# inferflow/inferflow

Measured on AMD Instinct MI355X. Metric: decode tokens/sec, Llama-2-7B Q4 batch=1 greedy (whole job), higher is better.
Workload: dtype i8 (Q8 activations x Q4_B32T1A weights, i32 dot, f32 scale, f16 I/O); 1 GPU; llama2_7b decode, Q4_B32T1A weights + F16 lm_head, F16 KV cache, batch 1 greedy, 16-token prompt, context 21..1851; parallelism=single, weights_bytes=4309647360

## Files before the change

inferflow_amd/csrc/ifa_decode_chain.h:

```cpp
#pragma once
#include "ifa_decode_kernels.h"

namespace ifa {

struct DecChainExtra {
    uint32_t *gran_a;
    uint32_t *gran_h;
    uint32_t *flags_a, *flags_h;
    const int *state;
    const unsigned *epoch;
    unsigned epoch_add;
    unsigned *err;
    int timeout_us;
    long long *trace;
    int late_w2;
};

__device__ __forceinline__ uint32_t chain_tag(unsigned call, int pos) { return 0x8000u | ((call & 127u) << 8) | ((unsigned)pos & 255u); }

typedef uint32_t ch_u32x4 __attribute__((ext_vector_type(4)));

template <int MAXC>
__device__ __forceinline__ bool chain_gather(half8_t (&xv)[MAXC], const uint32_t *gran, int cols, int nthr, uint32_t tag,
                                             long long t_give_up, unsigned *err, unsigned code)
// ... 152 lines not shown
        typename FmtA::W wo[RO];
        const int rows_o = PW.total_rows;
#pragma unroll
        for (int i = 0; i < RO; i++) {
            const int v = i * W + gw;
            if (i > 0 && v >= rows_o) continue;
            wo[i].load(PW.W0[0] + (size_t)min(v, rows_o - 1) * row_bytes_a, nblk_a, lane);
        }
        const half_t res = PW.residual[min(min(lane, RO - 1) * W + gw, rows_o - 1)];
        zero_ctl();
        read_tag();
        if (trf) { trc[0] = t_kernel; trc[1] = wall_clock64(); }
        __syncthreads();
        float aw[RO];
#pragma unroll
        for (int i = 0; i < RO; i++) aw[i] = (i == 0 || i * W + gw < rows_o) ? wo[i].dot(XA) : 0.0f;
#pragma unroll
        for (int i = 0; i < RO; i++) aw[i] = wave_sum(aw[i]);
        float a0 = 0.0f;
#pragma unroll
        for (int i = 0; i < RO; i++) { if (lane == i) a0 = aw[i]; }
        const int v = lane * W + gw;
        if (lane < RO && v < rows_o) {
            const DecRow d = dec_locate(PW, v);
            const half_t y = dec_row_value<EPI_RESIDUAL>(PW, d, a0, 0.0f, res, (half_t)0);
            chain_publish(E.gran_a, d.row, tag, y);
            d.y[d.row] = y;
        }
        chain_wave_published(ctl + CH_C_PUB_A, NW, E.flags_a + blockIdx.x, tag, lane);
        if (trf) trc[2] = wall_clock64();
        if (trl) trc[0] = wall_clock64();
        if (wave >= NP) {
            load_rows13(0, 0, RW);
        } else {
            if (wave == 0) { chain_poll_flags(E.flags_a, G, tag, lane, t_give_up, E.err, 0x93u); chain_go(ctl + CH_C_GO_A); }
            else lds_counter_wait(ctl + CH_C_GO_A, 1);
            chain_gather<MAXC>(pre.xv, E.gran_a, pcols, PT, tag, t_give_up, E.err, 0x91u);
            if (trf) trc[3] = wall_clock64();
            pre.finish(P.norm_w, P.norm_b, P.multi_base, P.eps, pcols, L, nullptr, nullptr);
            load_rows13(0, 0, RW);
        }
        lds_counter_wait(L.part + 131, NP);
    } else {
        if (threadIdx.x < PT) pre.issue(px, pnw, pnb, pcols);
        zero_ctl();
        if (NORM == 1 && wave >= NP) load_rows13(0, 0, 1);
        read_tag();
// ... 75 lines not shown
        else res = Q.residual[row];
        if (Q.residual2) res2 = Q.residual2[row];
    }
    if (trl) trc[3] = wall_clock64();
    lds_counter_wait(L2.part + 131, NP);
    if (trl) trc[4] = wall_clock64();
    if (lw >= rows2) return;
    float a2[R2];
#pragma unroll
    for (int i = 0; i < R2; i++) a2[i] = 0.0f;
#pragma unroll
    for (int j = 0; j < NJB; j++) {
        typename Fmt1::X Xj;
        Xj.load(L2.codes, L2.scale, L2.xsum, lane, nblk_b, 64 * j);
#pragma unroll
        for (int i = 0; i < R2; i++) a2[i] = (i == 0 || i * WL + lw < rows2) ? w2[i][j].dot(Xj, a2[i]) : 0.0f;
    }
#pragma unroll
    for (int i = 0; i < R2; i++) a2[i] = wave_sum(a2[i]);
    float b0 = 0.0f;
#pragma unroll
    for (int i = 0; i < R2; i++) { if (lane == i) b0 = a2[i]; }
    const int v2 = lane * WL + lw;
    if (lane < R2 && v2 < rows2) dec_finish_row<EPI_RESIDUAL>(Q, dec_locate(Q, v2), b0, 0.0f, res, res2);
    if (trl) trc[5] = wall_clock64();
}

bool dec_chain_supported(int w_dtype, int w2_dtype, int wo_dtype, int dim, int ffn, bool wo, int wo_cols, int num_cus);
int dec_chain_launch(int w_dtype, bool glu, int norm, bool wo, const DecGemvParams &P, const DecGemvParams &Q, const DecGemvParams *PW,
                     const DecChainExtra &E, int num_cus, hipStream_t s);
template <int DT>
int dec_chain_launch_dt(bool glu, int norm, bool wo, const DecGemvParams &P, const DecGemvParams &Q, const DecGemvParams &PW,
                        const DecChainExtra &E, int num_cus, hipStream_t s);

}
```

inferflow_amd/csrc/ifa_decode_kernels.h:

```cpp
#pragma once
#include "ifa_device.h"
#include "ifa_math.h"
#include "ifa_tiled.h"
#include "ifa_decode_formats.h"
#include "ifa_decode_gemv_plan.h"

namespace ifa {

typedef _Float16 half2_t __attribute__((ext_vector_type(2)));
typedef _Float16 half8_t __attribute__((ext_vector_type(8)));

__device__ __forceinline__ void q8_round_div8(const float (&v)[8], float qs, int (&q)[8])
{
    const float rqs = 1.0f / qs;
    bool risky = false;
#pragma unroll
    for (int i = 0; i < 8; i++) {
        const float t = v[i] * rqs;
        const float k = __builtin_rintf(t);
        risky |= fabsf(fabsf(t - k) - 0.5f) < 0.00006103515625f;
        q[i] = (int)k;
    }
    if (__builtin_expect(risky, 0)) {
#pragma unroll
// ... 6 lines not shown
#pragma unroll
    for (int i = 0; i < 8; i++) q[i] = min(max(q[i], -128), 127);
}

__device__ __forceinline__ int q8_round_div1(float v, float qs)
{
    if (qs <= 0.000001f) return 0;
    const float t = v * (1.0f / qs);
    float k = __builtin_rintf(t);
    if (__builtin_expect(fabsf(fabsf(t - k) - 0.5f) < 0.00006103515625f, 0)) k = roundf(v / qs);
    return min(max((int)k, -128), 127);
}

__device__ __forceinline__ void q8x4_dequant_h(uint32_t w, half2_t sc2, half2_t &lo, half2_t &hi)
{
    const uint32_t x = w ^ 0x80808080u;
    const uint32_t a = __builtin_amdgcn_perm(0x64646464u, x, 0x04010400u);
    const uint32_t b = __builtin_amdgcn_perm(0x64646464u, x, 0x04030402u);
    const half2_t bias = {(half_t)-1152.0f, (half_t)-1152.0f};
    lo = (__builtin_bit_cast(half2_t, a) + bias) * sc2;
    hi = (__builtin_bit_cast(half2_t, b) + bias) * sc2;
}

#ifndef IFA_NT_WEIGHTS
#define IFA_NT_WEIGHTS 1
#endif

struct XLds {
    int8_t *codes;
    float *scale;
    float *xsum;
    float *part;
    half_t *xh;
};


__device__ __forceinline__ XLds xlds_carve(char *smem, int cols)
{
    XLds l;
    size_t nb = (size_t)cols / 32;
    size_t off = 0;
    l.codes = reinterpret_cast<int8_t *>(smem); off += ((size_t)cols + 15) / 16 * 16;
    l.scale = reinterpret_cast<float *>(smem + off); off += nb * 4;
    l.xsum = reinterpret_cast<float *>(smem + off); off += nb * 4;
    off = (off + 15) / 16 * 16;
    l.part = reinterpret_cast<float *>(smem + off); off += 132 * 4;
// ... 57 lines not shown
#pragma unroll
            for (int i = 0; i < 8; i++) {
                half_t t = av[k][i];
                if (add_bias) t = f2h(h2f(t) + h2f(abv[k][i]));
                xv[k][i] = f2h(h2f(xv[k][i]) + h2f(t));
            }
            if (sum_out && blockIdx.x == 0) *reinterpret_cast<half8_t *>(sum_out + (size_t)c * 8) = xv[k];
        }
    }

    __device__ __forceinline__ void issue(const half_t *__restrict__ x, const half_t *__restrict__ nw,
                                          const half_t *__restrict__ nb, int cols)
    {
        const int chunks = cols >> 3;
#pragma unroll
        for (int k = 0; k < MAXC; k++) {
            const int c = threadIdx.x + k * nthr();
            if (c < chunks) {
                xv[k] = *reinterpret_cast<const half8_t *>(x + (size_t)c * 8);
                if constexpr (NORM == 1) {
                    if (nw) wv[k] = *reinterpret_cast<const half8_t *>(nw + (size_t)c * 8);
                    if (nb) bv[k] = *reinterpret_cast<const half8_t *>(nb + (size_t)c * 8);
                }
            }
        }
    }

    __device__ __forceinline__ void issue_norm(const half_t *__restrict__ nw, const half_t *__restrict__ nb, int cols)
    {
        if constexpr (NORM == 1) {
            const int chunks = cols >> 3;
#pragma unroll
            for (int k = 0; k < MAXC; k++) {
                const int c = threadIdx.x + k * nthr();
                if (c < chunks) {
                    if (nw) wv[k] = *reinterpret_cast<const half8_t *>(nw + (size_t)c * 8);
                    if (nb) bv[k] = *reinterpret_cast<const half8_t *>(nb + (size_t)c * 8);
                }
            }
        }
    }

    __device__ __forceinline__ void finish(const half_t *__restrict__ nw, const half_t *__restrict__ nb,
                                           float multi_base, float eps, int cols, const XLds &L,
                                           half_t *__restrict__ xn_out, long long *trc = nullptr)
    {
// ... 206 lines not shown

struct DecRow {
    int si, row;
    const uint8_t *W0, *W1;
    const half_t *b0, *b1;
    half_t *y;
};

__device__ __forceinline__ DecRow dec_locate(const DecGemvParams &P, int v)
{
    const int r0 = P.rows[0], r1 = P.rows[1];
    DecRow d;
    const bool in1 = P.nsets > 1 && v >= r0;
    const bool in2 = P.nsets > 2 && v >= r0 + r1;
    d.si = in2 ? 2 : (in1 ? 1 : 0);
    d.row = in2 ? v - r0 - r1 : (in1 ? v - r0 : v);
    d.W0 = in2 ? P.W0[2] : (in1 ? P.W0[1] : P.W0[0]);
    d.W1 = P.W1;
    d.b0 = in2 ? P.b0[2] : (in1 ? P.b0[1] : P.b0[0]);
    d.b1 = P.b1;
    d.y = in2 ? P.y[2] : (in1 ? P.y[1] : P.y[0]);
    return d;
}

template <int EPI>
__device__ __forceinline__ half_t dec_row_value(const DecGemvParams &P, const DecRow d, float a0, float a1, half_t res = (half_t)0,
                                                half_t res2 = (half_t)0)
{
    const int row = d.row;
    half_t y = dec_bias(a0, d.b0, row);
    if constexpr (EPI == EPI_RESIDUAL || EPI == EPI_PLAIN) {
        if (P.pre_scale != 0.0f) y = f2h(h2f(y) * P.pre_scale);
    }
    if constexpr (EPI == EPI_RESIDUAL) {
        y = f2h(h2f(res) + h2f(y));
        if (P.residual2) y = f2h(h2f(y) + h2f(res2));
        if (P.post_scale != 0.0f) y = f2h(h2f(y) * P.post_scale);
    } else if constexpr (EPI == EPI_GLU || EPI == EPI_MOE_GLU) {
        half_t t2 = dec_bias(a1, d.b1, row);
        half_t act = f2h(act_fn(h2f(y), P.act_kind));
        y = f2h(h2f(act) * h2f(t2));
    } else if constexpr (EPI == EPI_ACT || EPI == EPI_MOE_ACT) {
        y = f2h(act_fn(h2f(y), P.act_kind));
    } else if constexpr (EPI == EPI_MOE_ACC || EPI == EPI_MOE_LAST) {
        const half_t wexp = P.moe_w[P.moe_slot];
        const half_t prev = P.moe_slot == 0 ? (half_t)0 : P.moe_acc[row];
        y = __builtin_fmaf16(y, wexp, prev);
        if constexpr (EPI == EPI_MOE_LAST) {
            if (P.pre_scale != 0.0f) y = f2h(h2f(y) * P.pre_scale);
            y = f2h(h2f(y) + h2f(P.residual[row]));
            if (P.residual2) y = f2h(h2f(y) + h2f(P.residual2[row]));
            if (P.post_scale != 0.0f) y = f2h(h2f(y) * P.post_scale);
        }
    }
    return y;
}

template <int EPI>
__device__ __forceinline__ void dec_finish_row(const DecGemvParams &P, const DecRow d, float a0, float a1, half_t res = (half_t)0,
                                               half_t res2 = (half_t)0)
{
    d.y[d.row] = dec_row_value<EPI>(P, d, a0, a1, res, res2);
}

template <int DT, int NJ, int RW, int EPI, int NORM, bool XADD = false, int TH = DEC_THREADS, int NP = 0>
__global__ void __launch_bounds__(TH) k_dec_gemv(const half_t *px, const half_t *pnw, const half_t *pnb, int pcols,
                                                          const uint8_t *pw0, const uint8_t *pw1, int pnblk_grid, int ptotal,
                                                          const DecGemvParams P)
{
    extern __shared__ __attribute__((aligned(16))) char smem[];
    static_assert(NP == 0 || (NORM != 2 && !XADD && NP * 64 < TH), "wave-specialised prologue: a norm / quantiser prologue, some loader waves");
    constexpr int PT = NP ? NP * 64 : TH;
    constexpr int MAXC = NORM == 2 ? 1 : (NJ * 8 * block_capacity(DT) + PT - 1) / PT;
    XPre<NORM == 2 ? 0 : NORM, MAXC, XADD, NP * 64> pre;
    if constexpr (NORM != 2) {
        if (NP == 0 || threadIdx.x < PT) pre.issue(px, pnw, pnb, pcols);
        if constexpr (XADD) pre.issue_add(P.x_add, P.x_add_bias, pcols);
    }
    const long long t_start = wall_clock64();
    const XLds L = xlds_carve(smem, pcols);
    const int lane = threadIdx.x & 63;
    const int wave = __builtin_amdgcn_readfirstlane(threadIdx.x >> 6);
    const int gw = blockIdx.x * (TH / 64) + wave;
    const int W = (int)((unsigned)pnblk_grid >> 16) * (TH / 64);
    using Fmt = DecFmt<DT, NJ>;
    constexpr int NM = epi_is_glu(EPI) ? 2 : 1;
    const bool single = !epi_is_moe(EPI) && pw0 != nullptr;
    const int nblk_k = pnblk_grid & 0xFFFF, total_rows = ptotal;
    const size_t row_bytes = tiled_row_bytes(DT, (size_t)nblk_k);
    const int npass = (total_rows + RW * W - 1) / (RW * W);


    const uint8_t *moeW0 = nullptr, *moeW1 = nullptr, *moeW0b = nullptr, *moeW1b = nullptr, *moeW0c = nullptr, *moeW1c = nullptr;
    if constexpr (epi_is_moe(EPI)) {
        const int e = __builtin_amdgcn_readfirstlane(P.moe_sel[P.moe_slot]);
        moeW0 = P.w_table[4 * e + P.moe_tab_off];
        if constexpr (NM == 2) moeW1 = P.w_table[4 * e + P.moe_tab_off + 1];
        moeW0b = moeW0; moeW1b = moeW1; moeW0c = moeW0; moeW1c = moeW1;
        if (P.nsets > 1) {
            const int e1 = __builtin_amdgcn_readfirstlane(P.moe_sel[P.moe_slot + 1]);
            moeW0b = P.w_table[4 * e1 + P.moe_tab_off];
            if constexpr (NM == 2) moeW1b = P.w_table[4 * e1 + P.moe_tab_off + 1];
        }
        if (P.nsets > 2) {
            const int e2 = __builtin_amdgcn_readfirstlane(P.moe_sel[P.moe_slot + 2]);
            moeW0c = P.w_table[4 * e2 + P.moe_tab_off];
            if constexpr (NM == 2) moeW1c = P.w_table[4 * e2 + P.moe_tab_off + 1];
        }
    }
    auto moe_pick = [](int si, const uint8_t *a, const uint8_t *b, const uint8_t *c) { return si == 2 ? c : (si == 1 ? b : a); };
    typename Fmt::W w[NM][RW];
    auto load_rows = [&](int pass, int i0, int i1) {
        const bool full = (pass * RW + RW - 1) * W + gw < total_rows;
        auto one = [&](int i) {
            const int v = min((pass * RW + i) * W + gw, total_rows - 1);
            if (single) {
                w[0][i].load(pw0 + (size_t)v * row_bytes, nblk_k, lane);
                if constexpr (NM == 2) w[1][i].load(pw1 + (size_t)v * row_bytes, nblk_k, lane);
                return;
            }
            const DecRow d = dec_locate(P, v);
            const uint8_t *W0 = epi_is_moe(EPI) ? moe_pick(d.si, moeW0, moeW0b, moeW0c) : d.W0;
            w[0][i].load(W0 + (size_t)d.row * row_bytes, nblk_k, lane);
            if constexpr (NM == 2) { const uint8_t *W1 = epi_is_moe(EPI) ? moe_pick(d.si, moeW1, moeW1b, moeW1c) : d.W1; w[1][i].load(W1 + (size_t)d.row * row_bytes, nblk_k, lane); }
        };
        if (full) {
#pragma unroll
            for (int i = 0; i < RW; i++) { if (i < i0 || i >= i1) continue; one(i); }
        } else {
#pragma unroll
            for (int i = 0; i < RW; i++) {
                if (i < i0 || i >= i1) continue;
                if (i > 0 && (pass * RW + i) * W + gw >= total_rows) continue;
                one(i);
            }
        }
    };
    auto load_pass = [&](int pass) { load_rows(pass, 0, RW); };
    half_t res = (half_t)0, res2 = (half_t)0;
    auto load_epi = [&](int pass) {
        if constexpr (EPI == EPI_RESIDUAL) {
            const int v = min((pass * RW + min(lane, RW - 1)) * W + gw, total_rows - 1);
            const int row = single ? v : dec_locate(P, v).row;
            res = P.residual[row];
            if (P.residual2) res2 = P.residual2[row];
        }
    };
    constexpr int D1 = (NM * NJ * Fmt::DW >= 15) ? 1 : 2;

    typename Fmt::X X;
    bool tr = false;
    auto trace_on = [&]() { tr = P.trace != nullptr && threadIdx.x == 64; if (tr) P.trace[blockIdx.x * 8 + 0] = t_start; };
    if constexpr (NORM == 2) {
        const XqImage Q = xq_image_carve(const_cast<half_t *>(px), pcols);
        X.load(Q.codes, Q.scale, Q.xsum, lane, nblk_k);
        load_rows(0, 0, RW);
        load_epi(0);
        trace_on();
        if (tr) { P.trace[blockIdx.x * 8 + 1] = wall_clock64(); P.trace[blockIdx.x * 8 + 2] = wall_clock64(); }
        if (gw >= total_rows) return;
    } else {
        if constexpr (NP > 0) {
            if (threadIdx.x == TH - 1) { L.part[130] = 0.0f; L.part[131] = 0.0f; }
            constexpr int EARLY = NORM == 1 ? 1 : 0;
            if (EARLY && wave >= NP) load_rows(0, 0, 1);
            trace_on();
            __syncthreads();
            if (wave >= NP) {
                load_rows(0, EARLY, RW);
                load_epi(0);
                if (P.trace != nullptr && threadIdx.x == NP * 64 && NORM == 1) P.trace[blockIdx.x * 8 + 4] = wall_clock64();
            } else {
                if (tr) P.trace[blockIdx.x * 8 + 1] = wall_clock64();
                pre.finish(P.norm_w, P.norm_b, P.multi_base, P.eps, P.cols, L, P.xn_out,
                           (P.trace != nullptr && threadIdx.x == 0) ? P.trace + blockIdx.x * 8 : nullptr);
                load_rows(0, 0, RW);
                load_epi(0);
                if (tr) P.trace[blockIdx.x * 8 + 2] = wall_clock64();
            }
            lds_counter_wait(L.part + 131, NP);
        } else {
        __syncthreads();
        load_rows(0, 0, D1);
        trace_on();
        if (tr) P.trace[blockIdx.x * 8 + 1] = wall_clock64();
        if constexpr (XADD) pre.apply_add(P.x_add_bias, P.cols, P.xsum_out);
        pre.finish(P.norm_w, P.norm_b, P.multi_base, P.eps, P.cols, L, P.xn_out,
                   (P.trace != nullptr && threadIdx.x == 0) ? P.trace + blockIdx.x * 8 : nullptr);
        load_rows(0, D1, RW);
        load_epi(0);
        if (tr) P.trace[blockIdx.x * 8 + 2] = wall_clock64();
        }
        if (gw >= total_rows) return;
        X.load(L.codes, L.scale, L.xsum, lane, nblk_k);
    }
    if (tr) P.trace[blockIdx.x * 8 + 3] = wall_clock64();

    for (int pass = 0; pass < npass; pass++) {
        if (pass > 0) { load_pass(pass); load_epi(pass); }
        float a[NM][RW];
#pragma unroll
        for (int i = 0; i < RW; i++)
#pragma unroll
            for (int m = 0; m < NM; m++) a[m][i] = w[m][i].dot(X);
#pragma unroll
        for (int i = 0; i < RW; i++)
#pragma unroll
            for (int m = 0; m < NM; m++) a[m][i] = wave_sum(a[m][i]);
        float a0 = 0.0f, a1 = 0.0f;
#pragma unroll
        for (int i = 0; i < RW; i++) {
            if (lane == i) { a0 = a[0][i]; if constexpr (NM == 2) a1 = a[1][i]; }
        }
        const int v = (pass * RW + lane) * W + gw;
        if (lane < RW && v < total_rows) {
            dec_finish_row<EPI>(P, dec_locate(P, v), a0, a1, res, res2);
        }
    }
    if (tr) P.trace[blockIdx.x * 8 + 7] = wall_clock64();
}

template <int DT, int NJ, int RW, int EPI>
__global__ void __launch_bounds__(DEC_THREADS) k_dec_gemv_long(const DecGemvParams P)
{
    extern __shared__ __attribute__((aligned(16))) char smem[];
    const XLds L = xlds_carve(smem, P.cols);
    const int lane = threadIdx.x & 63;
    const int wave = __builtin_amdgcn_readfirstlane(threadIdx.x >> 6);
    const int gw = blockIdx.x * DEC_WAVES + wave;
    const int W = gridDim.x * DEC_WAVES;
    using Fmt = DecFmt<DT, NJ>;
    const size_t row_bytes = tiled_row_bytes(DT, (size_t)P.nblk);
    const int npass = (P.total_rows + RW * W - 1) / (RW * W);
    const int nchunk = (P.nblk + 64 * NJ - 1) / (64 * NJ);
    const int Q = npass * nchunk;
    const uint8_t *moeW0 = nullptr;
    if constexpr (epi_is_moe(EPI)) moeW0 = P.w_table[4 * __builtin_amdgcn_readfirstlane(P.moe_sel[P.moe_slot]) + P.moe_tab_off];
    typename Fmt::W wa[RW], wb[RW];
    auto load_q = [&](typename Fmt::W (&w)[RW], int q, int i0, int i1) {
        const int pass = q / nchunk, chunk = q - pass * nchunk;
#pragma unroll
        for (int i = 0; i < RW; i++) {
            if (i < i0 || i >= i1) continue;
            const int v = min((pass * RW + i) * W + gw, P.total_rows - 1);
            const DecRow d = dec_locate(P, v);
            const uint8_t *W0 = epi_is_moe(EPI) ? moeW0 : d.W0;
            w[i].load(W0 + (size_t)d.row * row_bytes, P.nblk, lane, chunk * 64 * NJ);
        }
    };
    {
        XPre<0, 8> pre;
        pre.issue(P.x, nullptr, nullptr, P.cols);
        __syncthreads();
        load_q(wa, 0, 0, 1);
        pre.finish(nullptr, nullptr, 0.0f, P.eps, P.cols, L, nullptr, nullptr);
        load_q(wa, 0, 1, RW);
    }
    if (gw >= P.total_rows) return;
    float a[RW];
#pragma unroll
    for (int i = 0; i < RW; i++) a[i] = 0.0f;
    auto compute = [&](typename Fmt::W (&w)[RW], int q) {
        const int pass = q / nchunk, chunk = q - pass * nchunk;
        typename Fmt::X X;
        X.load(L.codes, L.scale, L.xsum, lane, P.nblk, chunk * 64 * NJ);
#pragma unroll
        for (int i = 0; i < RW; i++) a[i] = w[i].dot(X, a[i]);
        if (chunk + 1 < nchunk) return;
#pragma unroll
        for (int i = 0; i < RW; i++) a[i] = wave_sum(a[i]);
        float a0 = 0.0f;
#pragma unroll
        for (int i = 0; i < RW; i++) { if (lane == i) a0 = a[i]; a[i] = 0.0f; }
        const int v = (pass * RW + lane) * W + gw;
        if (lane < RW && v < P.total_rows) {
            const DecRow d = dec_locate(P, v);
            half_t res = (half_t)0, res2 = (half_t)0;
            if constexpr (EPI == EPI_RESIDUAL) { res = P.residual[d.row]; if (P.residual2) res2 = P.residual2[d.row]; }
            dec_finish_row<EPI>(P, d, a0, 0.0f, res, res2);
        }
    };
    for (int q = 0; q < Q; q += 2) {
        if (q + 1 < Q) load_q(wb, q + 1, 0, RW);
        compute(wa, q);
        if (q + 1 < Q) {
            if (q + 2 < Q) load_q(wa, q + 2, 0, RW);
            compute(wb, q + 1);
        }
    }
}

struct DecLmHeadParams {
    const half_t *x;
    const half_t *norm_w, *norm_b;
    float multi_base, eps;
    int cols;
    const half_t *W;
    half_t *logits;
    int rows;
    half_t *xn_out;
};

// ... 177 lines not shown
```

inferflow_amd/csrc/ifa_dgemv_f16x.hip:

```cpp
#include "ifa_decode_gemv.h"
#include "ifa_codec.h"

namespace ifa {

constexpr int DH_ROWS = DEC_H_ROWS;

template <int DT>
struct HRow {
    const uint8_t *p;
    __device__ __forceinline__ float dot(const half_t *__restrict__ xs, int cols, int nblk, int lane) const
    {
        float acc = 0.0f;
        if constexpr (DT == F16) {
            const int chunks = cols >> 3;
            const u32x4 *w = reinterpret_cast<const u32x4 *>(p);
            const u32x4 *xv = reinterpret_cast<const u32x4 *>(xs);
            for (int c0 = lane; c0 < chunks; c0 += 256) {
                u32x4 wr[4];
#pragma unroll
                for (int j = 0; j < 4; j++) { const int c = c0 + 64 * j; wr[j] = w[min(c, chunks - 1)]; }
#pragma unroll
                for (int j = 0; j < 4; j++) { const int c = c0 + 64 * j; if (c < chunks) acc = dot8_f16(wr[j], xv[c], acc); }
            }
        } else {
// ... 57 lines not shown
            const int c = tid + k * DEC_THREADS;
            if (c >= chunks) continue;
            const half8_t v = *reinterpret_cast<const half8_t *>(xs + (size_t)c * 8);
            half8_t o;
#pragma unroll
            for (int i = 0; i < 8; i++) {
                float t = (float)v[i] * scale;
                if (P.norm_w) {
                    const float mlt = P.multi_base + h2f(P.norm_w[(size_t)c * 8 + i]);
                    t = t * mlt;
                    if (P.norm_b) t = t + h2f(P.norm_b[(size_t)c * 8 + i]);
                }
                o[i] = f2h(t);
            }
            *reinterpret_cast<half8_t *>(xs + (size_t)c * 8) = o;
            if (P.xn_out && blockIdx.x == 0) *reinterpret_cast<half8_t *>(P.xn_out + (size_t)c * 8) = o;
        }
        __syncthreads();
    }
    constexpr int NM = epi_is_glu(EPI) ? 2 : 1;
    const int gw = blockIdx.x * DEC_WAVES + wave;
    const int W = gridDim.x * DEC_WAVES;
    const size_t row_bytes = DT == F16 ? (size_t)P.cols * 2 : (size_t)P.nblk * block_bytes(DT);
    for (int v0 = gw; v0 < P.total_rows; v0 += DH_ROWS * W) {
        float a[NM][DH_ROWS];
#pragma unroll
        for (int i = 0; i < DH_ROWS; i++) {
            const int v = min(v0 + i * W, P.total_rows - 1);
            const DecRow d = dec_locate(P, v);
            HRow<DT> r0{d.W0 + (size_t)d.row * row_bytes};
            a[0][i] = r0.dot(xs, P.cols, P.nblk, lane);
            if constexpr (NM == 2) { HRow<DT> r1{d.W1 + (size_t)d.row * row_bytes}; a[1][i] = r1.dot(xs, P.cols, P.nblk, lane); }
        }
#pragma unroll
        for (int i = 0; i < DH_ROWS; i++)
#pragma unroll
            for (int mm = 0; mm < NM; mm++) a[mm][i] = wave_sum(a[mm][i]);
        float a0 = 0.0f, a1 = 0.0f;
#pragma unroll
        for (int i = 0; i < DH_ROWS; i++)
            if (lane == i) { a0 = a[0][i]; if constexpr (NM == 2) a1 = a[1][i]; }
        const int v = v0 + lane * W;
        if (lane < DH_ROWS && v < P.total_rows) {
            const DecRow d = dec_locate(P, v);
            half_t res = (half_t)0, res2 = (half_t)0;
            if constexpr (EPI == EPI_RESIDUAL) { res = P.residual[d.row]; if (P.residual2) res2 = P.residual2[d.row]; }
            dec_finish_row<EPI>(P, d, a0, a1, res, res2);
        }
    }
}

bool dec_gemv_h_supported(int w_dtype, size_t cols)
{
    return dec_gemv_h_cols_ok(w_dtype, cols);
}

DecGemvPlan dec_gemv_h_plan(const DecGemvFacts &f) { return plan_dec_gemv_h(f); }

template <int DT, int EPI, int NORM, bool XADD>
static int launch_h(const DecGemvParams &P, hipStream_t s)
{
    DecGemvFacts F;
    F.dtype = DT; F.epi = EPI; F.norm = NORM; F.x_add = XADD; F.cols = P.cols; F.total_rows = P.total_rows; F.num_cus = dec_num_cus();
    const DecGemvPlan R = plan_dec_gemv_h(F);
    if (R.error) return ifa_fail(IFA_ERR_ARG, "fused fp16-activation GEMV: dtype %d with %d columns is not supported", DT, P.cols);
    const size_t smem = (size_t)R.lds;
    const int wgs = R.grid;
    auto kern = k_dec_gemv_h<DT, EPI, NORM, XADD>;
    if (smem > 48 * 1024) IFA_HIP_CHECK(hipFuncSetAttribute((const void *)kern, hipFuncAttributeMaxDynamicSharedMemorySize, (int)smem));
    kern<<<dim3((unsigned)wgs), dim3(DEC_THREADS), smem, s>>>(P);
// ... 39 lines not shown
```

inferflow_amd/csrc/ifa_engine.hip:

```cpp
#include <mutex>
#include <unordered_map>
#include "ifa_engine_state.h"

namespace ifa {

namespace {
struct SpaceBook {
    std::mutex mu;
    std::unordered_map<void *, size_t> live;
    long long live_bytes = 0, fail_at = 0;
};
SpaceBook &book() { static SpaceBook *b = new SpaceBook(); return *b; }

template <class Alloc> int space_alloc(const char *call, void **p, size_t bytes, Alloc alloc)
{
    SpaceBook &b = book();
    *p = nullptr;
    {
        std::lock_guard<std::mutex> g(b.mu);
        if (b.fail_at > 0 && --b.fail_at == 0)
            return ifa_fail(IFA_ERR_HIP, "%s(%zu bytes) failed: out of memory (simulated: ifa_debug_alloc_fail_at)", call, bytes);
    }
    const hipError_t e = alloc(p, bytes);
    if (e != hipSuccess) {
// ... 89 lines not shown
        if (sl.exec) { (void)hipGraphExecDestroy(sl.exec); sl.exec = nullptr; }
        if (sl.graph) { (void)hipGraphDestroy(sl.graph); sl.graph = nullptr; }
    }
    for (auto &kv : m->batch_graphs) if (kv.second) (void)hipGraphExecDestroy(kv.second);
    m->batch_graphs.clear();
    for (auto &kv : m->draft_graphs) if (kv.second) (void)hipGraphExecDestroy(kv.second);
    m->draft_graphs.clear();
    sampled_drop_graphs(m);
}

int ensure_scratch(ifa_model *m, int T)
{
    if (T <= m->scratch_tokens) return IFA_OK;
    const ifa_model_config &c = m->cfg;
    const size_t D = c.dim, QD = (size_t)c.heads * c.head_dim, KVD = (size_t)c.kv_heads * c.head_dim, F = c.ffn;
    size_t maxcols = std::max(std::max(D, QD), F);
    Scratch n;
    int rc;
    if ((rc = n.x.alloc(T * D)) || (rc = n.x2.alloc(T * D)) || (rc = n.xn.alloc(T * D)) || (rc = n.hn.alloc(T * D)) || (rc = n.pn.alloc(T * D))
        || (rc = n.q.alloc(T * QD)) || (rc = n.k.alloc(T * KVD)) || (rc = n.v.alloc(T * KVD)) || (rc = n.att.alloc(T * QD))
        || (rc = n.a.alloc(T * D)) || (rc = n.f.alloc(T * D)) || (rc = n.t1.alloc(std::max<size_t>(T, 3) * F)) || (rc = n.t2.alloc(T * F))
        || (rc = n.logits.alloc((size_t)T * c.vocab)))
        return rc;
    if (!m->dqkv && (rc = n.dqkv.alloc(QD + 2 * KVD))) return rc;
    if (T <= 32 && !m->bqkv && ((rc = n.bqkv.alloc(32 * (QD + 2 * KVD))) || (rc = n.brope.alloc(32 * (size_t)c.head_dim)))) return rc;
    if (c.experts > 0) {
        const size_t cap = (size_t)T * (size_t)std::max(1, c.moe_top_k);
        if ((rc = n.moe_gate.alloc((size_t)T * c.experts)) || (rc = n.moe_out.alloc((size_t)T * D)) || (rc = n.moe_in.alloc((size_t)T * D))
            || (rc = n.moe_wdev.alloc(cap)) || (rc = n.moe_idx.alloc(cap)) || (rc = n.moe_pin.alloc(cap * (sizeof(int) + 2) + 16)))
            return rc;
        if (!m->moe_route) {
            if ((rc = n.moe_route.alloc(64 / sizeof(int)))) return rc;
            IFA_HIP_CHECK(hipMemsetAsync(n.moe_route, 0, 64, m->stream));
        }
        if ((rc = n.moe_sel.alloc(cap)) || (rc = n.moe_epos.alloc(cap)) || (rc = n.moe_counts.alloc(16))
            || (rc = n.moe_xq_in.alloc(cap * (D / 32 + 1) * 34)) || (rc = n.moe_xq_mid.alloc(cap * (F / 32 + 1) * 34))
            || (rc = n.moe_tiles.alloc((cap / 64 + (size_t)c.experts + 1) * sizeof(MoeTile)))
            || (rc = n.moe_singles.alloc(((size_t)c.experts + 1) * sizeof(MoeSingle))) || (rc = n.moe_smalls.alloc(((size_t)c.experts + 1) * sizeof(MoeTile)))
            || (rc = n.moe_selw.alloc(cap)) || (rc = n.moe_g1.alloc(cap * F)) || (rc = n.moe_g3.alloc(cap * F)) || (rc = n.moe_gin.alloc(cap * D))
            || (rc = n.moe_gout.alloc(cap * D)))
            return rc;
    }
    if ((rc = n.xq.alloc((maxcols / 32 + 1) * 34))) return rc;
    if (!m->attq && (rc = n.attq.alloc(xq_image_bytes(c.heads * c.head_dim)))) return rc;
    if ((rc = n.tokens_dev.alloc((size_t)T))) return rc;
    if (!n.dqkv) n.dqkv = std::move(m->dqkv);
    if (!n.bqkv) { n.bqkv = std::move(m->bqkv); n.brope = std::move(m->brope); }
// ... 447 lines not shown
}

int ifa_model_prompt_route(ifa_model *m, int *out, int n_out)
{
    IFA_REQUIRE(m && out && n_out >= PROMPT_ROUTE_N_OUT, "ifa_model_prompt_route: %d outputs expected", PROMPT_ROUTE_N_OUT);
    memcpy(out, &m->prompt_route, sizeof(m->prompt_route));
    return IFA_OK;
}

int ifa_model_get_buffer(ifa_model *m, const char *name, int layer, void **dptr, size_t *bytes)
{
    IFA_REQUIRE(m && name && dptr, "ifa_model_get_buffer: null pointer");
    const ifa_model_config &c = m->cfg;
    size_t b = 0; void *p = nullptr;
    if (!strcmp(name, "logits")) { p = m->logits; b = (size_t)c.vocab * 2; }
    else if (!strcmp(name, "logits_adj")) { p = m->la_adj; b = m->la_adj ? m->la_adj.cap() / m->g[T_LM_HEAD].rows * (size_t)c.vocab * 2 : 0; }
    else if (!strcmp(name, "logit_state")) { p = m->la_state; b = m->la_slots * m->g[T_LM_HEAD].rows * sizeof(unsigned); }
    else if (!strcmp(name, "tp_logits")) { p = m->tp_logits; b = m->tp_logits ? m->g[T_LM_HEAD].rows * 2 : 0; }
    else if (!strcmp(name, "trace")) { p = m->trace; b = m->trace ? sizeof(long long) * 2048 * 8 : 0; }
    else if (!strcmp(name, "hidden")) { p = m->xn; b = (size_t)c.dim * 2; }
    else if (!strcmp(name, "x")) { p = m->x; b = (size_t)c.dim * 2; }
    else if (!strcmp(name, "x2")) { p = m->x2; b = (size_t)c.dim * 2; }
    else if (!strcmp(name, "dqkv")) { p = m->dqkv; b = ((size_t)c.heads + 2 * (size_t)c.kv_heads) * c.head_dim * 2; }
    else if (!strcmp(name, "att")) { p = m->att; b = (size_t)c.heads * c.head_dim * 2; }
    else if (!strcmp(name, "attq")) { p = m->attq; b = m->attq ? xq_image_bytes(c.heads * c.head_dim) : 0; }
    else if (!strcmp(name, "a")) { p = m->a; b = (size_t)c.dim * 2; }
    else if (!strcmp(name, "t1")) { p = m->t1; b = (size_t)c.ffn * 2; }
    else if (!strcmp(name, "kcache") || !strcmp(name, "vcache")) {
        IFA_REQUIRE(layer >= 0 && layer < c.layers && m->finalized, "ifa_model_get_buffer: layer %d", layer);
        p = name[0] == 'k' ? m->layers[(size_t)layer].kcache : m->layers[(size_t)layer].vcache;
        b = m->kv_row_bytes * (size_t)c.max_ctx;
    } else return ifa_fail(IFA_ERR_ARG, "ifa_model_get_buffer: unknown buffer '%s'", name);
    *dptr = p;
    if (bytes) *bytes = b;
    return IFA_OK;
}

void *ifa_model_stream(ifa_model *m) { return m ? (void *)m->stream : nullptr; }

int ifa_model_set_stream(ifa_model *m, ifa_stream stream)
{
    IFA_REQUIRE(m, "ifa_model_set_stream: null model");
    IFA_HIP_CHECK(hipSetDevice(m->cfg.device));
    if (m->stream) IFA_HIP_CHECK(hipStreamSynchronize(m->stream));
    if (m->stream) (void)ifa_gemm_release_stream((ifa_stream)m->stream);
    if (m->stream && m->own_stream) IFA_HIP_CHECK(hipStreamDestroy(m->stream));
// ... 38 lines not shown
```

inferflow_amd/csrc/ifa_engine_state.h:

```cpp
#pragma once
#include <chrono>
#include <cstdlib>
#include <cstring>
#include <map>
#include <string>
#include <type_traits>
#include <vector>
#include "ifa_host.h"
#include "ifa_buf_hip.h"
#include "ifa_decode_kernels.h"
#include "ifa_decode_attn.h"
#include "ifa_decode_gemv.h"
#include "ifa_moe.h"
#include "ifa_gemm_rows_mfma.h"
#include "ifa_gemm_big.h"
#include "ifa_decode_lmhead_tail.h"
#include "ifa_decode_singles.h"
#include "ifa_decode_qkv_attn.h"
#include "ifa_decode_chain.h"
#include "ifa_prompt_route.h"

using namespace ifa;

namespace ifae {
// ... 6 lines not shown
       T_ATTN_POST_NORM = 29, T_ATTN_POST_NORM_B = 30, T_FFN_POST_NORM = 31, T_FFN_POST_NORM_B = 32,
       T_MAX = 36 };

struct Tensor {
    int dtype = -1;
    DevBuf<void> data;
    DevBuf<void> tiled;
    DevBuf<void> mo;
    DevBuf<void> q3hn;
    DevBuf<void> x32;
    size_t rows = 0, cols = 0;
    bool present() const { return data != nullptr; }
};

struct Layer {
    Tensor t[T_MAX];
    std::vector<Tensor> experts;
    DevBuf<void *> moe_table;
    DevBuf<void *> moe_table_aos;
    DevBuf<void *> moe_table_mo;
    DevBuf<void> kcache, vcache;
};

struct Scratch {
    DevBuf<half_t> x, x2, xn, hn, q, k, v;
    DevBuf<half_t> dqkv;
    DevBuf<half_t> bqkv;
    DevBuf<float> brope;
    DevBuf<half_t> att, a, f, t1, t2, logits;
    DevBuf<uint8_t> xq;
    DevBuf<int8_t> attq;
    DevBuf<half_t> moe_gate, moe_out;
    DevBuf<half_t> moe_in, moe_wdev;
    DevBuf<int> moe_route;
    DevBuf<int> moe_idx; PinBuf<void> moe_pin;
    DevBuf<int> moe_sel, moe_epos, moe_counts;
    DevBuf<half_t> moe_selw, moe_g1, moe_g3, moe_gin, moe_gout;
    DevBuf<uint8_t> moe_xq_in, moe_xq_mid;
    DevBuf<void> moe_tiles, moe_singles, moe_smalls;
    DevBuf<int> tokens_dev;
    DevBuf<half_t> pn;
};


}
using namespace ifae;
// ... 289 lines not shown
```

Baseline: 630.3 tokens/s.

## Read GEMV epilogue params from kernarg segment and branch-free row-set addressing

Reworks the decode GEMV epilogue and weight-row addressing. Parameters are read straight from the kernarg segment into scalar registers, and dec_locate is replaced with branch-free offset arithmetic. Bias and residual values are prefetched alongside the weight loads, and the unconditional clamped x issue (issue_all) removes per-chunk branches. It also adds a dqkv guard allocation so speculative reads stay in bounds, trace points, and a compile flag that disables the early-row prologue. The aim is to cut SGPR/VGPR pressure and the latency of the epilogue and prologue, at the cost of relying on a fixed kernarg layout and some extra clamped memory reads.

```diff
diff --git a/inferflow_amd/csrc/ifa_decode_chain.h b/inferflow_amd/csrc/ifa_decode_chain.h
--- a/inferflow_amd/csrc/ifa_decode_chain.h
+++ b/inferflow_amd/csrc/ifa_decode_chain.h
@@ -198,7 +198,7 @@
         for (int i = 0; i < RO; i++) { if (lane == i) a0 = aw[i]; }
         const int v = lane * W + gw;
         if (lane < RO && v < rows_o) {
-            const DecRow d = dec_locate(PW, v);
+            const DecRow d = dec_single(PW, v);
             const half_t y = dec_row_value<EPI_RESIDUAL>(PW, d, a0, 0.0f, res, (half_t)0);
             chain_publish(E.gran_a, d.row, tag, y);
             d.y[d.row] = y;
@@ -320,7 +320,7 @@
 #pragma unroll
     for (int i = 0; i < R2; i++) { if (lane == i) b0 = a2[i]; }
     const int v2 = lane * WL + lw;
-    if (lane < R2 && v2 < rows2) dec_finish_row<EPI_RESIDUAL>(Q, dec_locate(Q, v2), b0, 0.0f, res, res2);
+    if (lane < R2 && v2 < rows2) dec_finish_row<EPI_RESIDUAL>(Q, dec_single(Q, v2), b0, 0.0f, res, res2);
     if (trl) trc[5] = wall_clock64();
 }
 
diff --git a/inferflow_amd/csrc/ifa_decode_kernels.h b/inferflow_amd/csrc/ifa_decode_kernels.h
--- a/inferflow_amd/csrc/ifa_decode_kernels.h
+++ b/inferflow_amd/csrc/ifa_decode_kernels.h
@@ -52,6 +52,9 @@
     hi = (__builtin_bit_cast(half2_t, b) + bias) * sc2;
 }
 
+#ifndef IFA_GEMV_EARLY_ROW
+#define IFA_GEMV_EARLY_ROW 0
+#endif
 #ifndef IFA_NT_WEIGHTS
 #define IFA_NT_WEIGHTS 1
 #endif
@@ -155,6 +158,21 @@
                     if (nw) wv[k] = *reinterpret_cast<const half8_t *>(nw + (size_t)c * 8);
                     if (nb) bv[k] = *reinterpret_cast<const half8_t *>(nb + (size_t)c * 8);
                 }
+            }
+        }
+    }
+
+    __device__ __forceinline__ void issue_all(const half_t *__restrict__ x, const half_t *__restrict__ nw,
+                                              const half_t *__restrict__ nb, int cols)
+    {
+        const int chunks = cols >> 3;
+#pragma unroll
+        for (int k = 0; k < MAXC; k++) {
+            const int c = min((int)threadIdx.x + k * nthr(), chunks - 1);
+            xv[k] = *reinterpret_cast<const half8_t *>(x + (size_t)c * 8);
+            if constexpr (NORM == 1) {
+                if (nw) wv[k] = *reinterpret_cast<const half8_t *>(nw + (size_t)c * 8);
+                if (nb) bv[k] = *reinterpret_cast<const half8_t *>(nb + (size_t)c * 8);
             }
         }
     }
@@ -407,13 +425,85 @@
     d.y = in2 ? P.y[2] : (in1 ? P.y[1] : P.y[0]);
     return d;
 }
-
-template <int EPI>
-__device__ __forceinline__ half_t dec_row_value(const DecGemvParams &P, const DecRow d, float a0, float a1, half_t res = (half_t)0,
-                                                half_t res2 = (half_t)0)
-{
-    const int row = d.row;
-    half_t y = dec_bias(a0, d.b0, row);
+__device__ __forceinline__ DecRow dec_single(const DecGemvParams &P, int v)
+{
+    DecRow d;
+    d.si = 0; d.row = v;
+    d.W0 = P.W0[0]; d.W1 = P.W1;
+    d.b0 = P.b0[0]; d.b1 = P.b1;
+    d.y = P.y[0];
+    return d;
+}
+
+typedef __attribute__((address_space(1))) half_t g_half;
+typedef const __attribute__((address_space(4))) DecGemvParams DecGemvParamsK;
+template <int OFF>
+__device__ __forceinline__ DecGemvParamsK *dec_params_here()
+{
+    uint64_t a = (uint64_t)__builtin_amdgcn_kernarg_segment_ptr() + OFF;
+    asm volatile("" : "+s"(a));
+    return (DecGemvParamsK *)a;
+}
+struct DecEpi {
+    int r0, r1, nsets;
+    uint64_t y0, y1, y2, b00, b01, b02, bany;
+    const g_half *b1;
+    const g_half *residual, *residual2, *moe_w, *moe_acc;
+    int moe_slot, act_kind;
+    float pre_scale, post_scale;
+};
+__device__ __forceinline__ DecEpi dec_epi(DecGemvParamsK *K)
+{
+    DecEpi E;
+    DecGemvParamsK &P = *K;
+    uint64_t y0 = (uint64_t)P.y[0], y1 = (uint64_t)P.y[1], y2 = (uint64_t)P.y[2];
+    uint64_t b00 = (uint64_t)P.b0[0], b01 = (uint64_t)P.b0[1], b02 = (uint64_t)P.b0[2];
+    uint64_t b1 = (uint64_t)P.b1, rs = (uint64_t)P.residual, rs2 = (uint64_t)P.residual2, mw = (uint64_t)P.moe_w, ma = (uint64_t)P.moe_acc;
+    int r0 = P.rows[0], r1 = P.rows[1], ns = P.nsets, slot = P.moe_slot, act = P.act_kind;
+    float pre = P.pre_scale, post = P.post_scale;
+    asm volatile("" : "+s"(y0), "+s"(y1), "+s"(y2), "+s"(b00), "+s"(b01), "+s"(b02), "+s"(b1), "+s"(rs), "+s"(rs2), "+s"(mw), "+s"(ma));
+    asm volatile("" : "+s"(r0), "+s"(r1), "+s"(ns), "+s"(slot), "+s"(act), "+s"(pre), "+s"(post));
+    E.r0 = r0; E.r1 = r1; E.nsets = ns;
+    E.y0 = y0; E.y1 = y1; E.y2 = y2;
+    E.b00 = b00;
+    E.b01 = ns > 1 ? b01 : 0;
+    E.b02 = ns > 2 ? b02 : 0;
+    E.bany = E.b00 ? E.b00 : (E.b01 ? E.b01 : E.b02);
+    E.b1 = (const g_half *)b1;
+    E.residual = (const g_half *)rs; E.residual2 = (const g_half *)rs2;
+    E.moe_w = (const g_half *)mw; E.moe_acc = (const g_half *)ma;
+    E.moe_slot = slot; E.act_kind = act;
+    E.pre_scale = pre; E.post_scale = post;
+    return E;
+}
+struct DecOut {
+    int row;
+    g_half *y;
+    const g_half *b0;
+    int brow;
+    bool has_b0;
+};
+__device__ __forceinline__ DecOut dec_locate_out(const DecEpi &E, int v)
+{
+    const bool in1 = E.nsets > 1 && v >= E.r0;
+    const bool in2 = E.nsets > 2 && v >= E.r0 + E.r1;
+    const bool is1 = in1 && !in2;
+    DecOut o;
+    o.row = in2 ? v - E.r0 - E.r1 : (in1 ? v - E.r0 : v);
+    o.y = (g_half *)(E.y0 + (is1 ? E.y1 - E.y0 : 0) + (in2 ? E.y2 - E.y0 : 0));
+    const uint64_t b = E.b00 + (is1 ? E.b01 - E.b00 : 0) + (in2 ? E.b02 - E.b00 : 0);
+    o.has_b0 = b != 0;
+    o.b0 = (const g_half *)(o.has_b0 ? b : E.bany);
+    o.brow = o.has_b0 ? o.row : 0;
+    return o;
+}
+
+template <int EPI, class PP>
+__device__ __forceinline__ half_t dec_row_value_b(const PP &P, const int row, float a0, float a1, bool hb0, half_t bv0, bool hb1, half_t bv1,
+                                                  half_t res = (half_t)0, half_t res2 = (half_t)0)
+{
+    half_t y = f2h(a0);
+    if (hb0) y = f2h(h2f(y) + h2f(bv0));
     if constexpr (EPI == EPI_RESIDUAL || EPI == EPI_PLAIN) {
         if (P.pre_scale != 0.0f) y = f2h(h2f(y) * P.pre_scale);
     }
@@ -422,7 +512,8 @@
         if (P.residual2) y = f2h(h2f(y) + h2f(res2));
         if (P.post_scale != 0.0f) y = f2h(h2f(y) * P.post_scale);
     } else if constexpr (EPI == EPI_GLU || EPI == EPI_MOE_GLU) {
-        half_t t2 = dec_bias(a1, d.b1, row);
+        half_t t2 = f2h(a1);
+        if (hb1) t2 = f2h(h2f(t2) + h2f(bv1));
         half_t act = f2h(act_fn(h2f(y), P.act_kind));
         y = f2h(h2f(act) * h2f(t2));
     } else if constexpr (EPI == EPI_ACT || EPI == EPI_MOE_ACT) {
@@ -442,24 +533,57 @@
 }
 
 template <int EPI>
+__device__ __forceinline__ half_t dec_row_value(const DecGemvParams &P, const DecRow d, float a0, float a1, half_t res = (half_t)0,
+                                                half_t res2 = (half_t)0)
+{
+    half_t bv0 = (half_t)0, bv1 = (half_t)0;
+    if (d.b0) bv0 = d.b0[d.row];
+    if constexpr (EPI == EPI_GLU || EPI == EPI_MOE_GLU) { if (d.b1) bv1 = d.b1[d.row]; }
+    return dec_row_value_b<EPI>(P, d.row, a0, a1, d.b0 != nullptr, bv0, d.b1 != nullptr, bv1, res, res2);
+}
+
+template <int EPI>
+__device__ __forceinline__ void dec_epi_bias(const DecEpi &E, const DecOut &o, half_t &bv0, half_t &bv1)
+{
+    if (E.bany != 0) bv0 = o.b0[o.brow];
+    if constexpr (EPI == EPI_GLU || EPI == EPI_MOE_GLU) { if (E.b1 != nullptr) bv1 = E.b1[o.row]; }
+}
+
+template <int EPI>
+__device__ __forceinline__ void dec_finish_out(const DecEpi &E, const DecOut &o, float a0, float a1, half_t bv0, half_t bv1,
+                                               half_t res = (half_t)0, half_t res2 = (half_t)0)
+{
+    o.y[o.row] = dec_row_value_b<EPI>(E, o.row, a0, a1, o.has_b0, bv0, E.b1 != nullptr, bv1, res, res2);
+}
+
+template <int EPI>
 __device__ __forceinline__ void dec_finish_row(const DecGemvParams &P, const DecRow d, float a0, float a1, half_t res = (half_t)0,
                                                half_t res2 = (half_t)0)
 {
     d.y[d.row] = dec_row_value<EPI>(P, d, a0, a1, res, res2);
 }
 
+struct DecGemvLead {
+    const half_t *px, *pnw, *pnb;
+    int pcols;
+    const uint8_t *pw0, *pw1;
+    int pnblk_grid, ptotal;
+};
+static_assert(sizeof(DecGemvLead) == 56 && alignof(DecGemvParams) == 8 && sizeof(DecGemvLead) % alignof(DecGemvParams) == 0,
+              "k_dec_gemv: P follows its leading arguments without padding, at byte 56 of the argument segment");
 template <int DT, int NJ, int RW, int EPI, int NORM, bool XADD = false, int TH = DEC_THREADS, int NP = 0>
 __global__ void __launch_bounds__(TH) k_dec_gemv(const half_t *px, const half_t *pnw, const half_t *pnb, int pcols,
                                                           const uint8_t *pw0, const uint8_t *pw1, int pnblk_grid, int ptotal,
                                                           const DecGemvParams P)
 {
     extern __shared__ __attribute__((aligned(16))) char smem[];
+    constexpr int P_OFF = (int)sizeof(DecGemvLead);
     static_assert(NP == 0 || (NORM != 2 && !XADD && NP * 64 < TH), "wave-specialised prologue: a norm / quantiser prologue, some loader waves");
     constexpr int PT = NP ? NP * 64 : TH;
     constexpr int MAXC = NORM == 2 ? 1 : (NJ * 8 * block_capacity(DT) + PT - 1) / PT;
     XPre<NORM == 2 ? 0 : NORM, MAXC, XADD, NP * 64> pre;
     if constexpr (NORM != 2) {
-        if (NP == 0 || threadIdx.x < PT) pre.issue(px, pnw, pnb, pcols);
+        if (NP == 0 || threadIdx.x < PT) pre.issue_all(px, pnw, pnb, pcols);
         if constexpr (XADD) pre.issue_add(P.x_add, P.x_add_bias, pcols);
     }
     const long long t_start = wall_clock64();
@@ -493,43 +617,54 @@
             if constexpr (NM == 2) moeW1c = P.w_table[4 * e2 + P.moe_tab_off + 1];
         }
     }
-    auto moe_pick = [](int si, const uint8_t *a, const uint8_t *b, const uint8_t *c) { return si == 2 ? c : (si == 1 ? b : a); };
     typename Fmt::W w[NM][RW];
+    const uint8_t *wb0 = pw0, *wb1 = pw1;
+    uint64_t wd0b = 0, wd0c = 0, wd1b = 0, wd1c = 0;
+    int R0 = 0x7fffffff, R01 = 0x7fffffff;
+    auto sets_on = [&]() {
+        if (single) return;
+        if constexpr (epi_is_moe(EPI)) {
+            wb0 = moeW0; wd0b = (uint64_t)moeW0b - (uint64_t)moeW0; wd0c = (uint64_t)moeW0c - (uint64_t)moeW0;
+            if constexpr (NM == 2) { wb1 = moeW1; wd1b = (uint64_t)moeW1b - (uint64_t)moeW1; wd1c = (uint64_t)moeW1c - (uint64_t)moeW1; }
+        }
+        DecGemvParamsK &K = *dec_params_here<P_OFF>();
+        if constexpr (!epi_is_moe(EPI)) {
+            wb0 = K.W0[0]; wd0b = (uint64_t)K.W0[1] - (uint64_t)K.W0[0]; wd0c = (uint64_t)K.W0[2] - (uint64_t)K.W0[0];
+            if constexpr (NM == 2) wb1 = K.W1;
+        }
+        if (K.nsets > 1) R0 = K.rows[0];
+        if (K.nsets > 2) R01 = K.rows[0] + K.rows[1];
+    };
     auto load_rows = [&](int pass, int i0, int i1) {
-        const bool full = (pass * RW + RW - 1) * W + gw < total_rows;
-        auto one = [&](int i) {
-            const int v = min((pass * RW + i) * W + gw, total_rows - 1);
-            if (single) {
-                w[0][i].load(pw0 + (size_t)v * row_bytes, nblk_k, lane);
-                if constexpr (NM == 2) w[1][i].load(pw1 + (size_t)v * row_bytes, nblk_k, lane);
-                return;
-            }
-            const DecRow d = dec_locate(P, v);
-            const uint8_t *W0 = epi_is_moe(EPI) ? moe_pick(d.si, moeW0, moeW0b, moeW0c) : d.W0;
-            w[0][i].load(W0 + (size_t)d.row * row_bytes, nblk_k, lane);
-            if constexpr (NM == 2) { const uint8_t *W1 = epi_is_moe(EPI) ? moe_pick(d.si, moeW1, moeW1b, moeW1c) : d.W1; w[1][i].load(W1 + (size_t)d.row * row_bytes, nblk_k, lane); }
-        };
-        if (full) {
-#pragma unroll
-            for (int i = 0; i < RW; i++) { if (i < i0 || i >= i1) continue; one(i); }
-        } else {
-#pragma unroll
-            for (int i = 0; i < RW; i++) {
-                if (i < i0 || i >= i1) continue;
-                if (i > 0 && (pass * RW + i) * W + gw >= total_rows) continue;
-                one(i);
+#pragma unroll
+        for (int i = 0; i < RW; i++) {
+            if (i < i0 || i >= i1) continue;
+            const int vs = (pass * RW + i) * W + gw;
+            const int v = vs < total_rows ? vs : min(pass * RW * W + gw, total_rows - 1);
+            const bool in1 = v >= R0, in2 = v >= R01, is1 = in1 && !in2;
+            const int row = v - (is1 ? R0 : 0) - (in2 ? R01 : 0);
+            const uint8_t *W0 = wb0 + ((is1 ? wd0b : 0) + (in2 ? wd0c : 0));
+            w[0][i].load(W0 + (size_t)row * row_bytes, nblk_k, lane);
+            if constexpr (NM == 2) {
+                const uint8_t *W1 = wb1 + ((is1 ? wd1b : 0) + (in2 ? wd1c : 0));
+                w[1][i].load(W1 + (size_t)row * row_bytes, nblk_k, lane);
             }
         }
     };
     auto load_pass = [&](int pass) { load_rows(pass, 0, RW); };
-    half_t res = (half_t)0, res2 = (half_t)0;
+    half_t res = (half_t)0, res2 = (half_t)0, bv0 = (half_t)0, bv1 = (half_t)0;
+    DecEpi E;
+    auto epi_on = [&]() { E = dec_epi(dec_params_here<P_OFF>()); };
     auto load_epi = [&](int pass) {
+        const int v = min((pass * RW + min(lane, RW - 1)) * W + gw, total_rows - 1);
+        const DecOut o = dec_locate_out(E, v);
+        const g_half *some = (const g_half *)px;
         if constexpr (EPI == EPI_RESIDUAL) {
-            const int v = min((pass * RW + min(lane, RW - 1)) * W + gw, total_rows - 1);
-            const int row = single ? v : dec_locate(P, v).row;
-            res = P.residual[row];
-            if (P.residual2) res2 = P.residual2[row];
-        }
+            res = E.residual[o.row];
+            res2 = (E.residual2 ? E.residual2 : E.residual)[o.row];
+        }
+        bv0 = (E.bany != 0 ? o.b0 : some)[E.bany != 0 ? o.brow : 0];
+        if constexpr (epi_is_glu(EPI)) bv1 = (E.b1 != nullptr ? E.b1 : some)[E.b1 != nullptr ? o.row : 0];
     };
     constexpr int D1 = (NM * NJ * Fmt::DW >= 15) ? 1 : 2;
 
@@ -539,7 +674,9 @@
     if constexpr (NORM == 2) {
         const XqImage Q = xq_image_carve(const_cast<half_t *>(px), pcols);
         X.load(Q.codes, Q.scale, Q.xsum, lane, nblk_k);
+        sets_on();
         load_rows(0, 0, RW);
+        epi_on();
         load_epi(0);
         trace_on();
         if (tr) { P.trace[blockIdx.x * 8 + 1] = wall_clock64(); P.trace[blockIdx.x * 8 + 2] = wall_clock64(); }
@@ -547,26 +684,30 @@
     } else {
         if constexpr (NP > 0) {
             if (threadIdx.x == TH - 1) { L.part[130] = 0.0f; L.part[131] = 0.0f; }
-            constexpr int EARLY = NORM == 1 ? 1 : 0;
-            if (EARLY && wave >= NP) load_rows(0, 0, 1);
-            trace_on();
+            constexpr bool EARLY = IFA_GEMV_EARLY_ROW != 0 && NORM == 1;
+            if constexpr (EARLY) { sets_on(); if (wave >= NP) load_rows(0, 0, 1); }
             __syncthreads();
-            if (wave >= NP) {
-                load_rows(0, EARLY, RW);
-                load_epi(0);
-                if (P.trace != nullptr && threadIdx.x == NP * 64 && NORM == 1) P.trace[blockIdx.x * 8 + 4] = wall_clock64();
-            } else {
+            if constexpr (!EARLY) sets_on();
+            if (wave < NP) {
+                trace_on();
                 if (tr) P.trace[blockIdx.x * 8 + 1] = wall_clock64();
                 pre.finish(P.norm_w, P.norm_b, P.multi_base, P.eps, P.cols, L, P.xn_out,
                            (P.trace != nullptr && threadIdx.x == 0) ? P.trace + blockIdx.x * 8 : nullptr);
-                load_rows(0, 0, RW);
-                load_epi(0);
-                if (tr) P.trace[blockIdx.x * 8 + 2] = wall_clock64();
-            }
+            }
+            if (!EARLY || wave < NP) load_rows(0, 0, 1);
+            load_rows(0, 1, RW);
+            epi_on();
+            load_epi(0);
+            if (wave >= NP) { trace_on(); if (tr) P.trace[blockIdx.x * 8 + 1] = wall_clock64(); }
+            if (tr) P.trace[blockIdx.x * 8 + 2] = wall_clock64();
+            const bool tl = NORM == 1 && P.trace != nullptr && threadIdx.x == NP * 64;
             lds_counter_wait(L.part + 131, NP);
+            if (tl) P.trace[blockIdx.x * 8 + 4] = wall_clock64();
         } else {
         __syncthreads();
+        sets_on();
         load_rows(0, 0, D1);
+        epi_on();
         trace_on();
         if (tr) P.trace[blockIdx.x * 8 + 1] = wall_clock64();
         if constexpr (XADD) pre.apply_add(P.x_add_bias, P.cols, P.xsum_out);
@@ -582,7 +723,12 @@
     if (tr) P.trace[blockIdx.x * 8 + 3] = wall_clock64();
 
     for (int pass = 0; pass < npass; pass++) {
-        if (pass > 0) { load_pass(pass); load_epi(pass); }
+        if (pass > 0) {
+            load_pass(pass); load_epi(pass);
+            __builtin_amdgcn_sched_barrier(0);
+        }
+        const bool tt = tr && pass == npass - 1 && blockIdx.x < 1024;
+        if (tt) { asm volatile("s_waitcnt vmcnt(0)" ::: "memory"); P.trace[(1024 + blockIdx.x) * 8 + 5] = wall_clock64(); }
         float a[NM][RW];
 #pragma unroll
         for (int i = 0; i < RW; i++)
@@ -592,6 +738,7 @@
         for (int i = 0; i < RW; i++)
 #pragma unroll
             for (int m = 0; m < NM; m++) a[m][i] = wave_sum(a[m][i]);
+        if (tt) P.trace[(1024 + blockIdx.x) * 8 + 6] = wall_clock64();
         float a0 = 0.0f, a1 = 0.0f;
 #pragma unroll
         for (int i = 0; i < RW; i++) {
@@ -599,7 +746,7 @@
         }
         const int v = (pass * RW + lane) * W + gw;
         if (lane < RW && v < total_rows) {
-            dec_finish_row<EPI>(P, dec_locate(P, v), a0, a1, res, res2);
+            dec_finish_out<EPI>(E, dec_locate_out(E, v), a0, a1, bv0, bv1, res, res2);
         }
     }
     if (tr) P.trace[blockIdx.x * 8 + 7] = wall_clock64();
@@ -622,6 +769,7 @@
     const uint8_t *moeW0 = nullptr;
     if constexpr (epi_is_moe(EPI)) moeW0 = P.w_table[4 * __builtin_amdgcn_readfirstlane(P.moe_sel[P.moe_slot]) + P.moe_tab_off];
     typename Fmt::W wa[RW], wb[RW];
+    DecEpi E;
     auto load_q = [&](typename Fmt::W (&w)[RW], int q, int i0, int i1) {
         const int pass = q / nchunk, chunk = q - pass * nchunk;
 #pragma unroll
@@ -638,6 +786,7 @@
         pre.issue(P.x, nullptr, nullptr, P.cols);
         __syncthreads();
         load_q(wa, 0, 0, 1);
+        E = dec_epi(dec_params_here<0>());
         pre.finish(nullptr, nullptr, 0.0f, P.eps, P.cols, L, nullptr, nullptr);
         load_q(wa, 0, 1, RW);
     }
@@ -659,10 +808,11 @@
         for (int i = 0; i < RW; i++) { if (lane == i) a0 = a[i]; a[i] = 0.0f; }
         const int v = (pass * RW + lane) * W + gw;
         if (lane < RW && v < P.total_rows) {
-            const DecRow d = dec_locate(P, v);
-            half_t res = (half_t)0, res2 = (half_t)0;
-            if constexpr (EPI == EPI_RESIDUAL) { res = P.residual[d.row]; if (P.residual2) res2 = P.residual2[d.row]; }
-            dec_finish_row<EPI>(P, d, a0, 0.0f, res, res2);
+            const DecOut o = dec_locate_out(E, v);
+            half_t res = (half_t)0, res2 = (half_t)0, bv0 = (half_t)0, bv1 = (half_t)0;
+            if constexpr (EPI == EPI_RESIDUAL) { res = E.residual[o.row]; if (E.residual2) res2 = E.residual2[o.row]; }
+            dec_epi_bias<EPI>(E, o, bv0, bv1);
+            dec_finish_out<EPI>(E, o, a0, 0.0f, bv0, bv1, res, res2);
         }
     };
     for (int q = 0; q < Q; q += 2) {
diff --git a/inferflow_amd/csrc/ifa_dgemv_f16x.hip b/inferflow_amd/csrc/ifa_dgemv_f16x.hip
--- a/inferflow_amd/csrc/ifa_dgemv_f16x.hip
+++ b/inferflow_amd/csrc/ifa_dgemv_f16x.hip
@@ -103,6 +103,7 @@
     const int gw = blockIdx.x * DEC_WAVES + wave;
     const int W = gridDim.x * DEC_WAVES;
     const size_t row_bytes = DT == F16 ? (size_t)P.cols * 2 : (size_t)P.nblk * block_bytes(DT);
+    const DecEpi E = dec_epi(dec_params_here<0>());
     for (int v0 = gw; v0 < P.total_rows; v0 += DH_ROWS * W) {
         float a[NM][DH_ROWS];
 #pragma unroll
@@ -123,10 +124,11 @@
             if (lane == i) { a0 = a[0][i]; if constexpr (NM == 2) a1 = a[1][i]; }
         const int v = v0 + lane * W;
         if (lane < DH_ROWS && v < P.total_rows) {
-            const DecRow d = dec_locate(P, v);
-            half_t res = (half_t)0, res2 = (half_t)0;
-            if constexpr (EPI == EPI_RESIDUAL) { res = P.residual[d.row]; if (P.residual2) res2 = P.residual2[d.row]; }
-            dec_finish_row<EPI>(P, d, a0, a1, res, res2);
+            const DecOut o = dec_locate_out(E, v);
+            half_t res = (half_t)0, res2 = (half_t)0, bv0 = (half_t)0, bv1 = (half_t)0;
+            if constexpr (EPI == EPI_RESIDUAL) { res = E.residual[o.row]; if (E.residual2) res2 = E.residual2[o.row]; }
+            dec_epi_bias<EPI>(E, o, bv0, bv1);
+            dec_finish_out<EPI>(E, o, a0, a1, bv0, bv1, res, res2);
         }
     }
 }
diff --git a/inferflow_amd/csrc/ifa_engine.hip b/inferflow_amd/csrc/ifa_engine.hip
--- a/inferflow_amd/csrc/ifa_engine.hip
+++ b/inferflow_amd/csrc/ifa_engine.hip
@@ -135,7 +135,7 @@
         || (rc = n.a.alloc(T * D)) || (rc = n.f.alloc(T * D)) || (rc = n.t1.alloc(std::max<size_t>(T, 3) * F)) || (rc = n.t2.alloc(T * F))
         || (rc = n.logits.alloc((size_t)T * c.vocab)))
         return rc;
-    if (!m->dqkv && (rc = n.dqkv.alloc(QD + 2 * KVD))) return rc;
+    if (!m->dqkv && (rc = n.dqkv.alloc(QD + 2 * KVD + DQKV_GUARD))) return rc;
     if (T <= 32 && !m->bqkv && ((rc = n.bqkv.alloc(32 * (QD + 2 * KVD))) || (rc = n.brope.alloc(32 * (size_t)c.head_dim)))) return rc;
     if (c.experts > 0) {
         const size_t cap = (size_t)T * (size_t)std::max(1, c.moe_top_k);
@@ -629,6 +629,7 @@
     else if (!strcmp(name, "x")) { p = m->x; b = (size_t)c.dim * 2; }
     else if (!strcmp(name, "x2")) { p = m->x2; b = (size_t)c.dim * 2; }
     else if (!strcmp(name, "dqkv")) { p = m->dqkv; b = ((size_t)c.heads + 2 * (size_t)c.kv_heads) * c.head_dim * 2; }
+    else if (!strcmp(name, "dqkv_guard")) { p = m->dqkv ? m->dqkv + ((size_t)c.heads + 2 * (size_t)c.kv_heads) * c.head_dim : nullptr; b = m->dqkv ? DQKV_GUARD * 2 : 0; }
     else if (!strcmp(name, "att")) { p = m->att; b = (size_t)c.heads * c.head_dim * 2; }
     else if (!strcmp(name, "attq")) { p = m->attq; b = m->attq ? xq_image_bytes(c.heads * c.head_dim) : 0; }
     else if (!strcmp(name, "a")) { p = m->a; b = (size_t)c.dim * 2; }
diff --git a/inferflow_amd/csrc/ifa_engine_state.h b/inferflow_amd/csrc/ifa_engine_state.h
--- a/inferflow_amd/csrc/ifa_engine_state.h
+++ b/inferflow_amd/csrc/ifa_engine_state.h
@@ -52,6 +52,7 @@
     DevBuf<void> kcache, vcache;
 };
 
+constexpr size_t DQKV_GUARD = 16384;
 struct Scratch {
     DevBuf<half_t> x, x2, xn, hn, q, k, v;
     DevBuf<half_t> dqkv;
```

Measured after the change: 632.6 tokens/s (median of 3 runs). No clear change (+0.4%).
